# k2-fsa/Flow2GAN

Hardware: AMD Instinct MI355X
Metric: audio-seconds/sec (train step, G+D fwd/bwd) mel_24k_base (higher is better)
Workload: dtype f32 (fp32-class products on the bf16 matrix pipe for the long reductions and the direct MRD convs: every fp32 operand as three bf16 pieces = 24 significand bits, the six v_mfma_f32_32x32x16_bf16 products with i + j <= 2 per fp32 product, fp32 accumulate, error <= 2^-23 per product; short reductions ; 1 GPU; mel_24k_base GAN stage-2 train step: D-step + G-step, each on its own batch (MPD+MRD+FM+multi-scale mel), fwd+bwd+grad all-reduce, no optimizer (metric is fwd/bwd); per_gpu_batch=64, gan=gan_multi_scale_mel_recon, parallelism=dp1, optimizer=none

## Files before the change

flow2gan_amd/csrc/conv32x6.hip:

```cpp
#include <stdlib.h>

#include "conv32_common.h"

namespace {

typedef unsigned int u32x4 __attribute__((ext_vector_type(4)));

constexpr int NTAP = KH * KW;
constexpr int PB = 208;

__device__ __forceinline__ void split3(const f32x4 v, u32x2& p0, u32x2& p1, u32x2& p2) {
  unsigned a0, a1, a2, b0, b1, b2;
  f2g_split3_pair(v.x, v.y, a0, a1, a2);
  f2g_split3_pair(v.z, v.w, b0, b1, b2);
  p0 = u32x2{a0, b0};
  p1 = u32x2{a1, b1};
  p2 = u32x2{a2, b2};
}

__device__ __forceinline__ void store_px3(unsigned char* p, const f32x4 v) {
  u32x2 p0, p1, p2;
  split3(v, p0, p1, p2);
  *reinterpret_cast<u32x2*>(p) = p0;
  *reinterpret_cast<u32x2*>(p + 64) = p1;
// ... 502 lines not shown
      }
      if (row < XCH) split3(px_[row < XCH ? row : 0], kx[row < XCH ? row : 0][0], kx[row < XCH ? row : 0][1], kx[row < XCH ? row : 0][2]);
      if (row >= NK - GCH)
        split3(pg_[row >= NK - GCH ? row - (NK - GCH) : 0], kg[row >= NK - GCH ? row - (NK - GCH) : 0][0],
               kg[row >= NK - GCH ? row - (NK - GCH) : 0][1], kg[row >= NK - GCH ? row - (NK - GCH) : 0][2]);
    }
    {
      const int row = wave;
      bf16x8 a[3];
#pragma unroll
      for (int q = 0; q < 3; ++q) a[q] = tr_pix8(Gp + q * GPL + go + row * 16 * 64);
#pragma unroll
      for (int t = 0; t < 3; ++t) {
        bf16x8 b[3];
#pragma unroll
        for (int q = 0; q < 3; ++q) b[q] = tr_pix8(Xp + q * XPL + xs[t] + row * KR * IW * 64);
        mfma6(a, b, acc[3 + t]);
      }
    }
    __syncthreads();
    if (more) {
#pragma unroll
      for (int q = 0; q < XCH; ++q)
        if (xoff(q) >= 0) put3(Xp, XPL, xoff(q), kx[q]);
#pragma unroll
      for (int q = 0; q < GCH; ++q) put3(Gp, GPL, ((tid >> 3) + 64 * q) * 64 + c4 * 8, kg[q]);
    }
    __syncthreads();
  }
  static_assert(wgrad6_smem<TH, TW>() >= (size_t)8 * 16 * 64 * 4, "the flush reuses the planes as its reduction buffer");
  c32_wgrad_flush<NTAP, 3>(gw, reinterpret_cast<float*>(smb), acc, wave, lane, li, hh);
}

__global__ __launch_bounds__(512, 1) void conv33_x6_kernel(const f2g_conv32_desc d, int R, int tiles_h, int ntiles) {
  extern __shared__ __attribute__((aligned(16))) unsigned char smb[];
  unsigned char* At = smb;
  unsigned char* Bt = smb + P33 * PB;
  const int tid = threadIdx.x, lane = tid & 63, wave = tid >> 6;
  const int li = lane & 31, hh = lane >> 5;
  const int W = d.Win, PW = W + 2, npx = (R + 2) * PW, tpx = R * W;
  const unsigned mgW = magic_of(W), mgPW = magic_of(PW);
  {
    const unsigned char* wimg = reinterpret_cast<const unsigned char*>(d.w);
    for (int c = tid; c < T33 * C * 12; c += 512) {
      const int row = c / 12, part = c - row * 12;
      const int co = row / T33, tap = row - co * T33;
      *reinterpret_cast<u32x4*>(Bt + (tap * C + co) * PB + part * 16) =
          *reinterpret_cast<const u32x4*>(wimg + row * 192 + part * 16);
    }
  }
  constexpr int NQ = (P33 * 8 + 511) / 512;
  int prow[NQ], poff[NQ], pdst[NQ];
#pragma unroll
  for (int q = 0; q < NQ; ++q) {
    const int id = tid + 512 * q, px = id >> 3, c4 = id & 7;
    const int pr = fast_div(px, PW, mgPW), pc = px - pr * PW;
    const bool ok = px < npx && pc >= 1 && pc <= W;
    prow[q] = ok ? pr : -(1 << 20);
    poff[q] = (pr - 1) * (int)d.x_line + (pc - 1) * C + c4 * 4;
    pdst[q] = px < npx ? px * PB + c4 * 8 : -1;
  }
  auto load_patch = [&](int tile, f32x4 (&pf)[NQ]) {
    const int sq = tile / tiles_h, h0 = (tile - sq * tiles_h) * R;
    const float* org = d.x + (long long)sq * d.x_seq + (long long)h0 * d.x_line;
#pragma unroll
    for (int q = 0; q < NQ; ++q) {
      const int h = h0 - 1 + prow[q];
      pf[q] = *reinterpret_cast<const f32x4*>((h >= 0 && h < d.H) ? org + poff[q] : c32_zero);
    }
  };
  auto store_patch = [&](const f32x4 (&pf)[NQ]) {
#pragma unroll
    for (int q = 0; q < NQ; ++q)
      if (pdst[q] >= 0) store_px3(At + pdst[q], pf[q]);
  };
  const int mypx = wave * 32 + li;
  const int myr = fast_div(mypx, W, mgW), myc = mypx - myr * W;
  const unsigned char* Ap = At + (mypx < tpx ? ((myr + 1) * PW + myc + 1) * PB : (PW + 1) * PB) + hh * 16;
  const unsigned char* Bp = Bt + li * PB + hh * 16;
  const float bias = d.bias ? d.bias[li] : 0.f;
  float cs = 0.f;
  int tile = blockIdx.x;
  if (tile >= ntiles) return;
  {
    f32x4 pf[NQ];
    load_patch(tile, pf);
    store_patch(pf);
  }
  __syncthreads();
  for (; tile < ntiles; tile += gridDim.x) {
    const int nxt = tile + gridDim.x;
    const bool more = nxt < ntiles;
    f32x4 pf[NQ];
    load_patch(more ? nxt : tile, pf);
    const int sq = tile / tiles_h, h0 = (tile - sq * tiles_h) * R;
    const long long ybase = (long long)sq * d.y_seq + (long long)h0 * d.y_line;
    float my[16];
    if (d.mask_src) {
#pragma unroll
      for (int e = 0; e < 16; ++e) {
        const int p = wave * 32 + acc_row(e) + 4 * hh;
        const int r = fast_div(p, W, mgW), c = p - r * W;
        my[e] = (p < tpx && h0 + r < d.H) ? d.mask_src[ybase + (long long)r * d.y_line + c * C + li] : 1.f;
      }
    }
    f32x16 acc0, acc1;
#pragma unroll
    for (int e = 0; e < 16; ++e) { acc0[e] = 0.f; acc1[e] = 0.f; }
#pragma unroll
    for (int t = 0; t < T33; ++t)
      tap6(Ap + ((t / 3 - 1) * PW + (t % 3 - 1)) * PB, Bp + t * (C * PB), acc0, acc1);
    {
      float* ys = d.y + ybase;
#pragma unroll
      for (int e = 0; e < 16; ++e) {
        const int p = wave * 32 + acc_row(e) + 4 * hh;
        const int r = fast_div(p, W, mgW), c = p - r * W;
        if (p < tpx && h0 + r < d.H) {
          float v = acc0[e] + acc1[e] + bias;
          if (d.lrelu_slope != 0.f) v = v > 0.f ? v : d.lrelu_slope * v;
          if (d.mask_src) v *= my[e] > 0.f ? 1.f : d.mask_slope;
          cs += v;
          ys[(long long)r * d.y_line + c * C + li] = v;
        }
      }
    }
    __syncthreads();
    if (more) store_patch(pf);
    __syncthreads();
  }
  if (d.colsum) {
    cs += __shfl_xor(cs, 32);
    if (hh == 0) atomicAdd(d.colsum + li, cs);
  }
}


__global__ __launch_bounds__(512, 1) void conv33_wgrad6_kernel(const f2g_conv32_desc d, float* gw, int R,
                                                               int tiles_h, int ntiles) {
  extern __shared__ __attribute__((aligned(16))) unsigned char smb[];
  unsigned char* Xp = smb;
  unsigned char* Gp = smb + 3 * W33_XPL;
  const int tid = threadIdx.x, lane = tid & 63, wave = tid >> 6;
  const int li = lane & 31, hh = lane >> 5;
  const int W = d.Win, PW = W + 2, npx = (R + 2) * PW, ngp = R * PW, nks = (ngp + 15) >> 4;
  const unsigned mgPW = magic_of(PW);
  for (int o = tid * 16; o < 3 * (W33_XPL + W33_GPL); o += 512 * 16) *reinterpret_cast<u32x4*>(smb + o) = u32x4{0u, 0u, 0u, 0u};
  constexpr int NQ = (W33_GP * 8 + 511) / 512;
// ... 87 lines not shown
  const c32_tiling t = c32_pick_tiles(d->H, d->Wout);
  const long long nt = (long long)t.tiles_h * t.tiles_w * d->S;
  if (nt >= (1ll << 30) || d->x_line >= (1ll << 24)) return F2G_EINVAL;
  const int grid = (int)(nt < 256 ? nt : 256);
  return c32_launch_shape<conv32_s2_fwd6_kernel<8, 16>, conv32_s2_fwd6_kernel<16, 8>>(
      t.tall, fwd6_smem<8, 16>(), fwd6_smem<16, 8>(), dim3(grid), dim3(512), st, *d, t.tiles_w, t.tiles_h, (int)nt);
}

int f2g_conv32_dgrad6_launch(const f2g_conv32_desc* d, hipStream_t st) {
  const c32_tiling t = c32_pick_tiles(d->H, (d->Win + 1) / 2);
  const long long nt = (long long)t.tiles_h * t.tiles_w * d->S;
  if (nt >= (1ll << 30) || d->x_line >= (1ll << 24) || d->y_line >= (1ll << 24)) return F2G_EINVAL;
  const int grid = (int)(nt < 256 ? nt : 256);
  return c32_launch_shape<conv32_s2_dgrad6_kernel<8, 16>, conv32_s2_dgrad6_kernel<16, 8>>(
      t.tall, dgrad6_smem<8, 16>(), dgrad6_smem<16, 8>(), dim3(grid), dim3(512), st, *d, t.tiles_w, t.tiles_h,
      (int)nt);
}

int f2g_conv32_wgrad6_launch(const f2g_conv32_desc* d, float* gw, hipStream_t st) {
  const c32_tiling t = c32_pick_tiles(d->H, d->Wout);
  const long long nt = (long long)d->S * t.tiles_h * t.tiles_w;
  if (nt >= (1ll << 30) || d->x_line >= (1ll << 24)) return F2G_EINVAL;
  int per = (int)((nt + 255) / 256);
  if (per < 1) per = 1;
  const unsigned grid = (unsigned)((nt + per - 1) / per);
  return c32_launch_shape<conv32_s2_wgrad6_kernel<8, 16>, conv32_s2_wgrad6_kernel<16, 8>>(
      t.tall, wgrad6_smem<8, 16>(), wgrad6_smem<16, 8>(), dim3(grid), dim3(512), st, *d, gw, t.tiles_h, t.tiles_w,
      per);
}

int f2g_conv33_h3_launch(const f2g_conv32_desc* d, int R, int tiles_h, int ntiles, hipStream_t st);

extern "C" int f2g_conv33_fwd(const f2g_conv32_desc* d, f2g_stream_t stream) {
  if (!d || !d->x || !d->w || !d->y || (d->precision != 3 && d->precision != 4) || d->Win != d->Wout || d->fm_ref)
    return F2G_EINVAL;
  if ((((uintptr_t)d->x) & 15) || (((uintptr_t)d->w) & 15) || (d->x_line & 3) || (d->x_seq & 3)) return F2G_EINVAL;
  if (d->S <= 0 || d->H <= 0 || d->Win <= 0) return F2G_OK;
  const int W = d->Win;
  if (W > 112 || d->x_line >= (1ll << 24)) return F2G_EINVAL;
  if (d->y_line < (long long)W * C || (d->y != d->x && d->y_seq < (long long)d->H * d->y_line)) return F2G_EINVAL;
  if ((d->y_line & 3) || (d->y_seq & 3) || (((uintptr_t)d->y) & 15)) return F2G_EINVAL;
  if (d->mask_src && (d->lrelu_slope != 0.f || d->bias || (((uintptr_t)d->mask_src) & 15))) {
    f2g_set_error("f2g_conv33_fwd: mask_src (data-gradient role) excludes bias / lrelu_slope (forward role)");
    return F2G_EINVAL;
  }
  const int R = c33_pick_rows(d->H, W);
  if (R < 1) return F2G_EINVAL;
  const int tiles_h = (d->H + R - 1) / R;
  const long long nt = (long long)tiles_h * d->S;
  if (nt >= (1ll << 30)) return F2G_EINVAL;
  if (d->precision == 4) return f2g_conv33_h3_launch(d, R, tiles_h, (int)nt, (hipStream_t)stream);
  constexpr size_t smem = (size_t)P33 * PB + (size_t)T33 * C * PB;
  c32_lds_once<conv33_x6_kernel>(smem);
  const int grid = (int)(nt < 256 ? nt : 256);
  hipLaunchKernelGGL(conv33_x6_kernel, dim3(grid), dim3(512), smem, (hipStream_t)stream, *d, R, tiles_h, (int)nt);
  return f2g_check_launch();
}

extern "C" int f2g_conv33_wgrad(const f2g_conv32_desc* d, float* gw, f2g_stream_t stream) {
  if (!d || !d->x || !d->y || !gw || d->precision != 3 || d->Win != d->Wout) return F2G_EINVAL;
  if ((((uintptr_t)d->x) & 15) || (((uintptr_t)d->y) & 15) || (d->x_line & 3) || (d->x_seq & 3) || (d->y_line & 3) ||
      (d->y_seq & 3))
    return F2G_EINVAL;
  if (d->S <= 0 || d->H <= 0 || d->Win <= 0) return F2G_OK;
  const int W = d->Win;
  if (W > 112 || d->x_line >= (1ll << 24) || d->y_line >= (1ll << 24) || d->x_line < (long long)W * C ||
      d->y_line < (long long)W * C)
    return F2G_EINVAL;
  const int R = c33_pick_rows(d->H, W);
  if (R < 1) return F2G_EINVAL;
  const int tiles_h = (d->H + R - 1) / R;
  const long long nt = (long long)tiles_h * d->S;
  if (nt >= (1ll << 30)) return F2G_EINVAL;
  constexpr size_t smem = (size_t)3 * (W33_XPL + W33_GPL);
  static_assert(smem >= (size_t)8 * 16 * 64 * 4, "the flush reuses the planes as its reduction buffer");
  c32_lds_once<conv33_wgrad6_kernel>(smem);
  const int grid = (int)(nt < 256 ? nt : 256);
  hipLaunchKernelGGL(conv33_wgrad6_kernel, dim3(grid), dim3(512), smem, (hipStream_t)stream, *d, gw, R, tiles_h,
                     (int)nt);
  return f2g_check_launch();
}
```

flow2gan_amd/csrc/gemm_x6.hip:

```cpp
#include <stddef.h>
#include <stdint.h>

#include "gemm_common.h"
#include "x6_epilogue.h"

#define X6_MFMA_PRIO 1

#if F2G_X6LAB & 256
__device__ unsigned long long g_x6prof[8];
extern "C" int f2g_lab_x6prof(unsigned long long* out8) {
  unsigned long long z[8] = {0, 0, 0, 0, 0, 0, 0, 0};
  if (hipMemcpyFromSymbol(out8, HIP_SYMBOL(g_x6prof), sizeof(z)) != hipSuccess) return 1;
  return hipMemcpyToSymbol(HIP_SYMBOL(g_x6prof), z, sizeof(z)) != hipSuccess;
}
#endif

__global__ __launch_bounds__(256) void split3_img_kernel(__bf16* __restrict__ dst, const float* __restrict__ src,
                                                         long long ld, long long rows, int K) {
  const long long total = rows * (K / 4);
  for (long long i = (long long)blockIdx.x * blockDim.x + threadIdx.x; i < total;
       i += (long long)gridDim.x * blockDim.x) {
    const long long r = i / (K / 4);
    const int k4 = (int)(i - r * (K / 4)) * 4;
    const float4 v = *reinterpret_cast<const float4*>(src + r * ld + k4);
    const float x[4] = {v.x, v.y, v.z, v.w};
    unsigned short p[3][4];
#pragma unroll
    for (int e = 0; e < 4; ++e) {
      const __bf16 a = (__bf16)x[e];
      const float r1 = x[e] - (float)a;
      const __bf16 b = (__bf16)r1;
      const __bf16 c = (__bf16)(r1 - (float)b);
      p[0][e] = __builtin_bit_cast(unsigned short, a);
      p[1][e] = __builtin_bit_cast(unsigned short, b);
      p[2][e] = __builtin_bit_cast(unsigned short, c);
    }
// ... 518 lines not shown
#pragma unroll
    for (int ks = 0; ks < 2; ++ks)
#pragma unroll
      for (int sdeg = 2; sdeg >= 0; --sdeg)
#pragma unroll
        for (int i = 0; i < 3; ++i) {
          const int j = sdeg - i;
          if (j < 0 || j > 2) continue;
          acc[0][0] = __builtin_amdgcn_mfma_f32_32x32x16_bf16(fa[ks][i], fb[ks][j], acc[0][0], 0, 0, 0);
        }
  }
  const f2g_epilogue& E = d.E;
  if (E.aux || E.res || E.prelu_slope || E.atomic || E.accumulate || E.scale != 0.f) {
    gemm_epilogue<1, 1>(E, acc, M, N, m0, n0, wave, 0, li, h, true);
    return;
  }
  __syncthreads();
  long long* rowoff = reinterpret_cast<long long*>(smem6);
  if (tid < 128) {
    const int row = m0 + tid;
    long long off = -1;
    if (row < M) {
      if (E.P0o > 0) {
        const int sq = row / E.P0o;
        off = (long long)sq * E.seq_stride_o + (long long)(row - sq * E.P0o) * E.row_stride_o + E.off_o;
      } else {
        off = (long long)row * E.ldc;
      }
    }
    rowoff[tid] = off;
  }
  __syncthreads();
  const int col = li;
  if (col >= N) return;
  const float bias = E.bias ? E.bias[col] : 0.f;
  const float fmw = E.fm_ref ? E.fm_w * (E.fm_wdev ? E.fm_wdev[0] : 1.f) : 0.f;
  float cs = 0.f;
#pragma unroll
  for (int e = 0; e < 16; ++e) {
    const long long ro = rowoff[wave * 32 + (e & 3) + 8 * (e >> 2) + 4 * h];
    if (ro < 0) continue;
    const long long off = ro + col;
    float v = acc[0][0][e] + bias;
    if (E.lrelu_slope != 0.f) v = v > 0.f ? v : E.lrelu_slope * v;
    if (E.mask_src) {
      const float y = E.mask_src[off];
      if (E.fm_ref) {
        const float dl = y - E.fm_ref[off];
        v += fmw * (dl > 0.f ? 1.f : (dl < 0.f ? -1.f : 0.f));
      }
      v *= y > 0.f ? 1.f : E.mask_slope;
    }
    cs += v;
    E.C[off] = v;
  }
  if (E.colsum) {
    cs += __shfl_xor(cs, 32);
    if (h == 0) atomicAdd(E.colsum + col, cs);
  }
}


static bool x6_shape_ok(const f2g_gemm_desc& d) {
  if (d.form != 0 || !host_plain(d.B) || d.A.cols != d.B.cols) return false;
  const long long M = d.A.rows, N = d.B.rows, K = d.A.cols, ext = x6_a_extent(d.A);
  if (K < 32 || (K % 32) || M < 1 || N < 1 || ext <= 0) return false;
  if (ext * 6 >= 0xe0000000ll || N * K * 6 >= 0xe0000000ll) return false;
  if (d.A.alpha || d.A.lrelu_src || d.B.alpha || d.B.lrelu_src) return false;
  if (d.E.c_bf16 || d.E.atomic || d.split_k > 1) return false;
  if (d.E.x3_out) {
    const f2g_epilogue& E = d.E;
    if (E.prelu_out || (((uintptr_t)E.x3_out) & 15) || (((uintptr_t)E.C) & 15) || (N % 8)) return false;
    if (E.P0o > 0 ? ((E.seq_stride_o | E.row_stride_o | E.off_o) & 7) != 0 : (E.ldc & 7) != 0) return false;
  }
  return true;
}

static int x6_wide(const f2g_gemm_desc& d) {
  return x6e::wide_ok(d.E, d.B.rows) ? 1 : 0;
}

static bool x6f_ok(const f2g_gemm_desc& d) {
  if (d.A.split || (d.B.split != 0 && d.B.split != 3 && d.B.split != 4) || !x6_shape_ok(d)) return false;
  if (d.B.split == 4 && ((d.B.rows & 31) || d.B.rows <= 32 || d.B.P0 != 1 || d.B.P1 != 1)) return false;
  if (!al16(d.A.base) || !al16(d.B.base) || (d.A.seq_stride & 3) || (d.B.split == 0 && (d.B.seq_stride & 3))) return false;
  const long long ext = host_plain(d.A) ? (long long)d.A.rows * d.A.seq_stride : x6_a_extent(d.A);
  return ext * 4 < 0xe0000000ll && (long long)d.B.rows * (d.B.split ? d.B.cols * 6ll : d.B.seq_stride * 4) < 0xe0000000ll;
}

// ... 57 lines not shown
      f2g_note_kernel("x6n", 1, 5);
      hipLaunchKernelGGL(gemm_x6n_kernel, dim3((M + 127) / 128), dim3(256), smem_n, st, d, M, N, K, x6_rows_of(d.A, 4));
      break;
    }
    case X6_G: {
      constexpr size_t smem_g = 4 * x6e::ESZ > 128 * 208 ? 4 * x6e::ESZ : 128 * 208;
      f2g_note_kernel("x6g", 1, 4);
      hipLaunchKernelGGL(gemm_x6g_kernel, grid, dim3(256), smem_g, st, d, M, N, K, x6_rows_of(d.A, 4), x6_wide(d));
      break;
    }
    case X6_F:
      dyn_lds_once<gemm_x6f_kernel<false>, gemm_x6f_kernel<true>>((int)smem);
      f2g_note_kernel(pick.arg ? "x6f<wimg=1>" : "x6f<wimg=0>", 1, 4);
      hipLaunchKernelGGL(pick.arg ? gemm_x6f_kernel<true> : gemm_x6f_kernel<false>, grid, dim3(256), smem, st, d, M, N,
                         K, x6_rows_of(d.A, 4), x6_wide(d));
      break;
  }
  return f2g_check_launch();
}

extern "C" int f2g_gemm_x6_ok(const f2g_gemm_desc* d) {
  if (!d || !x6_shape_ok(*d)) return 0;
  return 1 | ((x6_tap_ok(*d, 5) || x6_tap_ok(*d, 2)) ? 2 : 0) | (x6f_ok(*d) ? 4 : 0);
}

extern "C" int32_t f2g_gemm_colsum_part_rows(const f2g_gemm_desc* dp) {
  if (!dp || (dp->precision != 3 && dp->precision != 4) || dp->form != 0) return 0;
  f2g_gemm_desc d = *dp;
  if (d.E.colsum_part_ld <= 0) d.E.colsum_part_ld = 4;
  if (d.precision == 4) {
    const int tile = f2g_gemm_h3_part_tile(d);
    return tile ? tile / 64 * ((d.A.rows + tile - 1) / tile) : 0;
  }
  if (!x6_wide(d)) return 0;
  const int M = d.A.rows;
  switch (x6_choose(d).kind) {
    case X6_NONE:
    case X6_N:
      return 0;
    case X6_P:
      return 4 * ((M + 255) / 256);
    default:
      return 2 * ((M + 127) / 128);
  }
}

extern "C" int64_t f2g_split_bf16x3_bytes(int32_t rows, int32_t K) { return (int64_t)rows * K * 6; }

extern "C" int f2g_split_bf16x3(void* dst, const float* src, int64_t ld, int32_t rows, int32_t K,
                                f2g_stream_t stream) {
  if (!dst || !src || rows < 0 || K < 32 || (K % 32) || ld < K || (ld & 3) || (((uintptr_t)src) & 15) ||
      (((uintptr_t)dst) & 15))
    return F2G_EINVAL;
  if (rows == 0) return F2G_OK;
  const long long total = (long long)rows * (K / 4);
  hipLaunchKernelGGL(split3_img_kernel, dim3(f2g_grid_for(total, 256)), dim3(256), 0, (hipStream_t)stream,
                     reinterpret_cast<__bf16*>(dst), src, (long long)ld, (long long)rows, K);
  return f2g_check_launch();
}
```

flow2gan_amd/csrc/thin_epilogue.h:

```cpp
#pragma once
#include "common.h"

namespace thin {

typedef float f32x16 __attribute__((ext_vector_type(16)));

__device__ __forceinline__ void row_offsets(const f2g_epilogue& E, int M, int m0, int tid, long long* rowoff) {
  if (tid >= 128) return;
  const int row = m0 + tid;
  long long off = -1;
  if (row < M) {
    if (E.P0o > 0) {
      const int sq = row / E.P0o;
      off = (long long)sq * E.seq_stride_o + (long long)(row - sq * E.P0o) * E.row_stride_o + E.off_o;
    } else {
      off = (long long)row * E.ldc;
    }
  }
  rowoff[tid] = off;
}

__device__ __forceinline__ float row_values(const f2g_epilogue& E, const f32x16& acc, int N, int wave, int li, int h,
                                            const long long* rowoff) {
  const int col = li;
// ... 24 lines not shown

__device__ __forceinline__ float row_values_cut(const f2g_epilogue& E, const f32x16& acc, int rg, int col0, int li,
                                                int h, const long long* rowoff, const int* rowlive) {
  const int col = col0 + li;
  float cs = 0.f;
  const float fmw = E.fm_ref ? E.fm_w * (E.fm_wdev ? E.fm_wdev[0] : 1.f) : 0.f;
#pragma unroll
  for (int e = 0; e < 16; ++e) {
    const int tr = rg * 32 + (e & 3) + 8 * (e >> 2) + 4 * h;
    const long long ro = rowoff[tr];
    if (ro < 0 || col >= rowlive[tr]) continue;
    const long long off = ro + col;
    float v = acc[e];
    if (E.mask_src) {
      const float y = E.mask_src[off];
      if (E.fm_ref) {
        const float dl = y - E.fm_ref[off];
        v += fmw * (dl > 0.f ? 1.f : (dl < 0.f ? -1.f : 0.f));
      }
      v *= y > 0.f ? 1.f : E.mask_slope;
    }
    cs += v;
    E.C[off] = v;
  }
  return cs;
}

__device__ __forceinline__ void column_sums(const f2g_epilogue& E, int N, int li, int h, float cs) {
  if (!E.colsum) return;
  cs += __shfl_xor(cs, 32);
  if (h == 0 && li < N) atomicAdd(E.colsum + li, cs);
}

}
```

flow2gan_amd/fused_disc.py:

```python
from __future__ import annotations

from typing import List

import torch

from . import ops
from .fused import deliver_grads, filterbank_spec, filterbank_spec_bwd, sink_register
from .models.modules import dft_matrices
from .ops import gemm, mat, win1d, win2d

SLOPE = 0.1


def stack_pair(real, fake):
    B, T = real.shape
    x2 = ops.empty(2 * B, T, device=real.device)
    ops.copy3(x2, 0, T, real.contiguous(), 0, T, 1, B, T)
    ops.copy3(x2, 0, T, fake.contiguous(), 0, T, 1, B, T, out_offset=B * T)
    return x2


def pack_conv_weight(w):
    Cout, Cin, kh, kw = w.shape
    out = ops.empty(Cout, kh * kw * Cin, device=w.device)
# ... 22 lines not shown
MPD_CH = (1, 32, 128, 512, 1024, 1024)
MPD_STRIDE = (3, 3, 3, 3, 1)


def mpd_params(mpd) -> list:
    p = []
    for d in mpd.discriminators:
        for c in d.convs:
            p += [c.weight, c.bias]
        p += [d.conv_post.weight, d.conv_post.bias]
    return p


HALO = 2


def _halo_rows(S: int, H: int, Cc: int, dev, x3: bool = False):
    buf = ops.empty(S * (H + 2 * HALO), Cc, device=dev)
    if Cc % 4 == 0:
        ops.zero_halo(buf, S, H + 2 * HALO, Cc, HALO, HALO)
    else:
        ops.fill_(buf, 0.0)
    if x3:
        ops.x3_reserve(buf, (S, H + 2 * HALO, Cc, HALO, HALO))
    return buf


def _halo_map(H: int, Cc: int):
    return (H, (H + 2 * HALO) * Cc, Cc, HALO * Cc)


def unhalo(y, S: int, H: int):
    return y.view(S, H + 2 * HALO, y.shape[1])[:, HALO:HALO + H]


def _mpd_forward_one(x2, p: int, prm: list, keep_images: bool = False):
    dev = x2.device
    S2, T = x2.shape
    H = (T + p - 1) // p
    S = S2 * p
    img = ops.empty(S * H, 1, device=dev)
    ops.period_fold(img, x2, S2, T, p, H)
    acts, hs = [img], [H]
    shares = [None] * 6
    x = img
    for l in range(5):
        w, b = prm[2 * l], prm[2 * l + 1]
        Cin, Cout, st = MPD_CH[l], MPD_CH[l + 1], MPD_STRIDE[l]
        Hout = (H + 4 - 5) // st + 1
        wp = ops.derived(w, "pack", pack_conv_weight)
        y = _halo_rows(S, Hout, Cout, dev, x3=(0 < l < 4))
        if l == 0:
            ops.mpd0_fwd(x, S, H, Hout, HALO, w.reshape(Cout, 5), b, SLOPE, y)
        else:
            A = win1d(x, S, H + 2 * HALO, Cin, Hout, st, 0, 5)
            if keep_images:
                shares[l] = ops.split_sharing(x)
                with shares[l]:
                    gemm(A, mat(wp), y, bias=b, lrelu=SLOPE, rowmap=_halo_map(Hout, Cout), x3_out=(l < 4))
            else:
                gemm(A, mat(wp), y, bias=b, lrelu=SLOPE, rowmap=_halo_map(Hout, Cout), x3_out=(l < 4))
        acts.append(y)
        hs.append(Hout)
        x, H = y, Hout
    wpost, bpost = prm[10], prm[11]
    wpp = ops.derived(wpost, "pack", pack_conv_weight)
    scores = ops.empty(S * H, 1, device=dev)
    ops.mpdpost_fwd(x, S, H, HALO, wpp, bpost, scores)
    return dict(acts=acts, hs=hs, scores=scores, S=S, p=p, shares=shares)


def _dgrad_weight(w, stride: int, j0: int, nt: int):
    def build(t):
        Cout, Cin, K = t.shape[0], t.shape[1], t.shape[2] * t.shape[3]
        out = ops.empty(Cin, nt * Cout, device=t.device)
        ops.permute4(out, t, (Cin, nt, Cout, 1), (K, -stride, Cin * K, 0),
                     in_offset=j0 + stride * (nt - 1))
        return out
    return ops.derived(w, ("dgradT", stride, j0, nt), build)


def _dgrad_weight3(w):
    def build(t):
        Cout, Cin, K = t.shape[0], t.shape[1], t.shape[2] * t.shape[3]
        out = ops.empty(3 * Cin, 2 * Cout, device=t.device)
        ops.fill_(out[:Cin], 0.0)
        one = ops.empty(Cin, Cout, device=t.device)
        ops.permute4(one, t, (Cin, 1, Cout, 1), (K, -3, Cin * K, 0), in_offset=2)
        ops.copy3(out, 2 * Cout, 0, one, Cout, 0, Cin, 1, Cout)
        for rho in (1, 2):
            ops.permute4(out[rho * Cin:(rho + 1) * Cin], t, (Cin, 2, Cout, 1), (K, -3, Cin * K, 0), in_offset=rho + 2)
        return out
    return ops.derived(w, ("dgradT3", 3), build)

# ... 9 lines not shown


def _conv1d_dgrad(g_pre, S, Hout, Cout, w, stride, pad, Hin, mask=None, fm=None, colsum=None):
    Cin, K = w.shape[1], w.shape[2] * w.shape[3]
    dev = g_pre.device
    want_img = 2 * Cin >= ops.X6_MIN_K
    gx = _halo_rows(S, Hin, Cin, dev, x3=want_img)
    if (K, stride, pad, Cin, Cout) == (5, 3, 2, 32, 128) and not want_img \
            and _conv1d_dgrad3(g_pre, S, Hout, Cout, w, Hin, gx, mask, fm, colsum):
        return gx
    for rho, j0, nt, e0, Lq in _residues(K, stride, pad, Hin):
        if Lq == 0:
            continue
        wq = _dgrad_weight(w, stride, j0, nt)
        wpad = (nt - 1) - e0
        A = win1d(g_pre, S, Hout + 2 * HALO, Cout, Lq, 1, wpad - HALO, nt)
        rm = (Lq, (Hin + 2 * HALO) * Cin, stride * Cin, (HALO + rho) * Cin)
        gemm(A, mat(wq), gx, rowmap=rm, mask=mask, fm=fm, colsum=colsum, x3_out=want_img)
    return gx


class MPDFusedLanding:

    def __init__(self, st, Sx: int, roff: int, g1, train_disc: bool):
        self.acts, self.hs, self.Sx, self.roff, self.g1, self.train_disc = st["acts"], st["hs"], Sx, roff, g1, train_disc

    def __call__(self, l_out, producer, cs):
        y, Sx, g1 = self.acts[l_out], self.Sx, self.g1
        Hp_, C_ = self.hs[l_out] + 2 * HALO, y.shape[1]
        mk = (y, self.roff * Hp_ * C_, SLOPE)
        fk = None
        if (not self.train_disc) and l_out >= 2:
            fk = (y, 0, 1.0 / (Sx * self.hs[l_out] * C_), g1)
        if l_out == 5 or (ops.GEMM_PRECISION == 3 and l_out in (3, 4)):
            return producer(mk, fk, cs)
        gm = producer(None, None, None)
        gm._f2g_x3_bad = True
        n_ = Sx * Hp_ * C_
        if self.train_disc:
            ops.lrelu_bwd_colsum(gm, y, None, 0.0, SLOPE, Sx * Hp_, C_, C_, cs, y_off=mk[1])
        elif fk is not None:
            ops.lrelu_bwd(gm, y, y, fk[2], SLOPE, 1, n_, n_, wdev=g1, y_off=mk[1], r_off=0)
        else:
            ops.lrelu_bwd(gm, y, None, 0.0, SLOPE, 1, n_, n_, y_off=mk[1])
        return gm


class MPDUpstreamLanding:

    def __init__(self, st, B: int, ups: dict):
        self.acts, self.hs, self.S, self.p, self.B, self.ups = st["acts"], st["hs"], st["S"], st["p"], B, ups

    def __call__(self, l_out, producer, cs):
        gm = producer(None, None, None)
        gm._f2g_x3_bad = True
        y, Hl, p = self.acts[l_out], self.hs[l_out], self.p
        Hp_, C_ = Hl + 2 * HALO, y.shape[1]
        u = self.ups.get(l_out)
        if u is not None:
            ub, uc, uh, uw = u.stride()
            ops.lrelu_bwd_add(gm, y, (self.B, p, Hl), (p * Hp_ * C_, Hp_ * C_, C_), C_, u, (ub, uw, uh, uc),
                              SLOPE, colsum=cs, g_off=HALO * C_)
        elif cs is not None:
            ops.lrelu_bwd_colsum(gm, y, None, 0.0, SLOPE, self.S * Hp_, C_, C_, cs)
        else:
            n_ = self.S * Hp_ * C_
            ops.lrelu_bwd(gm, y, None, 0.0, SLOPE, 1, n_, n_)
        return gm


# ... 233 lines not shown
                y = None
                gemm(A, mat(wp), cat, bias=b, lrelu=SLOPE,
                     rowmap=(Wout, Wcat * MRD_CH, MRD_CH, foff * MRD_CH))
            layer_out.append(y)
            x, x_is_spec = y, False
        acts.append(layer_out)
    wpost, bpost = prm[50], prm[51]
    scores = ops.empty(S * Ft * Wcat, 1, device=dev)
    w9 = ops.derived(wpost, "pack", pack_conv_weight)
    if ops.GEMM_PRECISION in (0, 1, 3):
        ops.convpost_fwd(cat, S, Ft, Wcat, w9, bpost, scores)
    else:
        gemm(win2d(cat, S, Ft, Wcat, MRD_CH, Wcat, 3, 3, 1, 1, 1), mat(w9), scores, bias=bpost)
    return dict(xn=xn, stats=stats, packed=packed, ldp=ldp, Ft=Ft, nb=nb, hop=hop, bands=bands,
                widths=widths, Wcat=Wcat, cat=cat, acts=acts, scores=scores)


def _conv2d_dgrad(g_pre, S, H, Wout, Cout, w, sw, Win, gx, *, g_line=None, g_seq=None, g_off=0,
                  x_line=None, x_off=0, mask=None, fm=None, colsum=None):
    Cin, kh, kw = w.shape[1], w.shape[2], w.shape[3]
    dev = g_pre.device
    pw = kw // 2
    if (ops.GEMM_PRECISION in (0, 1, 3) and Cin == MRD_CH and Cout == MRD_CH and kw == 9
            and sw == 2 and x_line is None and x_off == 0):
        def build_t(t):
            out = ops.empty(kh * kw, Cin, Cout, device=t.device)
            ops.permute4(out, t, (kh * kw, Cin, Cout, 1), (1, kh * kw, Cin * kh * kw, 0))
            return out
        wT = ops.derived(w, "dgrad_taps", build_t)
        ops.conv32_s2_dgrad(g_pre, S, H, Win, Wout, wT, gx, g_seq=g_seq, g_line=g_line, g_off=g_off,
                            mask=mask, fm=fm, colsum=colsum)
        return gx
    if (ops.GEMM_PRECISION == 3 and Cin == MRD_CH and Cout == MRD_CH
            and kh == 3 and kw == 3 and sw == 1 and x_line is None and x_off == 0 and fm is None
            and Win <= ops.CONV33_MAX_W):
        def build_f(t):
            out = ops.empty(Cin, kh * kw * Cout, device=t.device)
            ops.permute4(out, t, (Cin, kh * kw, Cout, 1), (kh * kw, -1, Cin * kh * kw, 0), in_offset=kh * kw - 1)
            return out
        wf = ops.derived(w, "dgrad33", build_f)
        ops.conv33(g_pre, S, H, Win, wf, None, 0.0, gx, x_off=g_off, x_line=g_line, x_seq=g_seq, form=1,
                   mask=mask, colsum=colsum)
        return gx
    if x_line is None:
        x_line = Win * Cin
    for rho, j0, ntw, e0, Lq in _residues(kw, sw, pw, Win):
        if Lq == 0:
            continue
        def build(t, j0=j0, ntw=ntw):
            out = ops.empty(kh * ntw * Cout, Cin, device=t.device)
            ops.permute4(out, t, (kh, ntw, Cout, Cin), (-kw, -sw, Cin * kh * kw, kh * kw),
                         in_offset=(kh - 1) * kw + j0 + sw * (ntw - 1))
            return out
        wq = ops.derived(w, ("dgrad2d", sw, j0, ntw), build)
        A = win2d(g_pre, S, H, Wout, Cout, Lq, kh, ntw, 1, 1, (ntw - 1) - e0, line_stride=g_line,
                  seq_stride=g_seq, offset=g_off)
        gemm(A, mat(wq), gx, form=1, rowmap=(Lq, x_line, sw * Cin, x_off + rho * Cin), mask=mask,
             fm=fm, colsum=colsum)
    return gx


def _mrd_foffs(st) -> list:
    foffs, foff = [], 0
    for ws in st["widths"]:
        foffs.append(foff)
        foff += ws[5]
    return foffs


class MRDFusedLanding:
    fused = True

    def __init__(self, st, Sx: int, soff: int, g1, train_disc: bool):
        self.st, self.Sx, self.soff, self.g1, self.train_disc = st, Sx, soff, g1, train_disc
        self.foffs = _mrd_foffs(st)

    def __call__(self, bi, l_out, producer, cs):
        st, Sx, soff, g1, train_disc = self.st, self.Sx, self.soff, self.g1, self.train_disc
        Ft, C = st["Ft"], MRD_CH
        Wl = st["widths"][bi][l_out + 1]
        if l_out == 4:
            gcat, cat, ldc, foff = producer(None, None, None), st["cat"], st["Wcat"] * C, self.foffs[bi]
            y_off = soff * Ft * ldc + foff * C
            if train_disc:
                ops.lrelu_bwd(gcat, cat, None, 0.0, SLOPE, Sx * Ft, Wl * C, ldc, g_off=foff * C, y_off=y_off)
            else:
                ops.lrelu_bwd(gcat, cat, cat, 1.0 / (Sx * Ft * Wl * C), SLOPE, Sx * Ft, Wl * C, ldc,
                              wdev=g1, g_off=foff * C, y_off=y_off, r_off=foff * C)
            return gcat
        yb = st["acts"][bi][l_out]
        nb_ = Sx * Ft * Wl * C
        mk = (yb, soff * Ft * Wl * C, SLOPE)
        fmk = (yb, 0, 1.0 / nb_, g1) if ((not train_disc) and l_out >= 1) else None
        if (train_disc and ops.GEMM_PRECISION == 3 and ops.CONV32_X6
                and (l_out < 3 or Wl <= ops.CONV33_MAX_W)):
            return producer(mk, fmk, cs)
        gx = producer(None, None, None)
        if train_disc:
            ops.lrelu_bwd_colsum(gx, yb, None, 0.0, SLOPE, Sx * Ft * Wl, C, C, cs, y_off=mk[1])
        elif fmk is not None:
            ops.lrelu_bwd(gx, yb, yb, fmk[2], SLOPE, 1, nb_, nb_, wdev=g1, y_off=mk[1], r_off=0)
        else:
            ops.lrelu_bwd(gx, yb, None, 0.0, SLOPE, 1, nb_, nb_, y_off=mk[1])
        return gx


class MRDUpstreamLanding:
    fused = False

    def __init__(self, st, S: int, g_maps):
        self.st, self.S, self.g_maps = st, S, g_maps
        self.foffs = _mrd_foffs(st)

    def __call__(self, bi, l_out, producer, cs):
        st, S = self.st, self.S
        Ft, C = st["Ft"], MRD_CH
        Wl = st["widths"][bi][l_out + 1]
        gm = producer(None, None, None)
        u = self.g_maps[4 * bi + l_out - 1] if l_out >= 1 else None
        if l_out == 4:
            y, line, off = st["cat"], st["Wcat"] * C, self.foffs[bi] * C
        else:
            y, line, off = st["acts"][bi][l_out], Wl * C, 0
        if u is not None:
            ub, uc, uf, uw = u.stride()
            ops.lrelu_bwd_add(gm, y, (S, Ft, Wl), (Ft * line, line, C), C, u, (ub, uf, uw, uc), SLOPE,
                              colsum=cs, g_off=off)
        elif l_out == 4:
            ops.lrelu_bwd(gm, y, None, 0.0, SLOPE, S * Ft, Wl * C, line, g_off=off, y_off=off)
            if cs is not None:
# ... 272 lines not shown
```

flow2gan_amd/ops.py:

```python
from __future__ import annotations

import ctypes as C
from typing import Callable, NamedTuple, Optional

import torch

from . import _lib as L
from ._opts import opt
from ._lib import DwconvBwd, DwnormBwd, DwnormFwd, Epilogue, GemmDesc, Operand, call, ptr


def empty(*shape, device, dtype=torch.float32):
    return torch.empty(*shape, device=device, dtype=dtype)


def zeros(*shape, device):
    t = torch.empty(*shape, device=device, dtype=torch.float32)
    fill_(t, 0.0)
    return t


def fill_(t, v: float):
    if BATCH is not None and t.numel() > 0:
        import struct
# ... 910 lines not shown
            continue
        d.precision = 4
        if mark_a:
            d.A.split = mark_a
        if mark_b:
            d.B.split = mark_b
        ask = lambda: L.lib.f2g_gemm_f16_ok(C.byref(d)) == needs
        if _ask_with_x3_out(d, out, out_offset, x3_out, prelu_out, ask) if wide else ask():
            return r
        if mark_a or mark_b:
            d.A.split = d.B.split = 0
    return None


def _fp16x3_gemm(d, A, Bm, out, form: int, atomic: bool, split_k: int, out_offset: int, x3_out: bool,
                 prelu_out) -> bool:
    r = _fp16x3_route(d, A, Bm, out, form, atomic, split_k, out_offset, x3_out, prelu_out)
    if r is None:
        return False
    image_a, image_b = r.images
    new_a = image_a(A) if image_a is not None else None
    new_b = image_b(Bm) if image_b is not None else None
    if new_a is not None:
        d.A = new_a
    if new_b is not None:
        d.B = new_b
    globals()[r.counter] += 1
    if x3_out and r.x3_out and d.E.x3_out:
        out._f2g_x3 = out._f2g_x3_buf
    return True


CONV32_X6 = opt("conv32_x6", True)


def x3_image(t2d):
    def build(t):
        rows, K = t.shape
        img = torch.empty(rows * K * 3, device=t.device, dtype=torch.bfloat16)
        split3(img, t, 0, K, rows, K)
        return img
    return derived(t2d, "x3img", build) if _is_const(t2d) else build(t2d)


def _timed_conv(name, flops, shape, *args):
    if GEMM_TIMER is not None:
        GEMM_TIMER.time(lambda: call(name, *args), flops, shape)
    else:
        call(name, *args)


FP16X3_CONV32_FWD = opt("fp16x3_conv32_fwd", False)
FP16X3_CONV32_DGRAD = opt("fp16x3_conv32_dgrad", False)
FP16X3_CONV32_WGRAD = opt("fp16x3_conv32_wgrad", False)
FP16X3_CONV33_FWD = opt("fp16x3_conv33_fwd", False)
FP16X3_CONV33_DGRAD = opt("fp16x3_conv33_dgrad", False)
FP16X3_CONV33_WGRAD = opt("fp16x3_conv33_wgrad", False)
FP16X3_CONV32_FWD_LAUNCHES = 0
FP16X3_CONV32_DGRAD_LAUNCHES = 0
FP16X3_CONV32_WGRAD_LAUNCHES = 0
FP16X3_CONV33_FWD_LAUNCHES = 0
FP16X3_CONV33_DGRAD_LAUNCHES = 0
FP16X3_CONV33_WGRAD_LAUNCHES = 0


def conv32_f16_image(w):
# ... 4 lines not shown

def _conv32_operand(d, w, rows_k=None, h3: bool = False):
    img = w
    if GEMM_PRECISION == 1:
        d.precision = 1
        img = derived(w, "split", split_bf16) if w is not None else None
    elif GEMM_PRECISION == 3 and CONV32_X6:
        if h3 and FP16X3 and w is not None:
            d.precision = 4
            img = conv32_f16_image(w)
        else:
            d.precision = 3
            img = x3_image(w.view(rows_k) if rows_k else w) if w is not None else None
    if img is not w:
        d._keep = img
    return img


def conv32_s2_fwd(x, S: int, H: int, Win: int, Wout: int, w_packed, bias, slope: float, y):
    global FP16X3_CONV32_FWD_LAUNCHES
    d = L.Conv32Desc()
    d.x, d.x_seq, d.x_line = ptr(x), H * Win * 32, Win * 32
    d.S, d.H, d.Win, d.Wout = S, H, Win, Wout
    d.w, d.bias, d.lrelu_slope = ptr(_conv32_operand(d, w_packed, h3=FP16X3_CONV32_FWD)), ptr(bias), slope
    FP16X3_CONV32_FWD_LAUNCHES += d.precision == 4
    d.y, d.y_seq, d.y_line = ptr(y), H * Wout * 32, Wout * 32
    _timed_conv("f2g_conv32_s2_fwd", 2.0 * S * H * Wout * 32 * 27 * 32, (0, S * H * Wout, 32, 27 * 32), C.byref(d))
    return y


CONV33_MAX_W = 112


def conv33(x, S: int, H: int, W: int, w_packed, bias, slope: float, y, x_off: int = 0, x_line=None, x_seq=None,
           y_off: int = 0, y_line=None, y_seq=None, form: int = 0, mask=None, colsum=None):
    global FP16X3_CONV33_FWD_LAUNCHES, FP16X3_CONV33_DGRAD_LAUNCHES
    d = L.Conv32Desc()
    d.x = ptr(x) + 4 * x_off
    d.x_line = x_line if x_line is not None else W * 32
    d.x_seq = x_seq if x_seq is not None else H * d.x_line
    d.S, d.H, d.Win, d.Wout = S, H, W, W
    if FP16X3 and GEMM_PRECISION == 3 and CONV32_X6 and (FP16X3_CONV33_DGRAD if form == 1 else FP16X3_CONV33_FWD):
        img = conv32_f16_image(w_packed)
        d.precision = 4
        if form == 1:
            FP16X3_CONV33_DGRAD_LAUNCHES += 1
        else:
            FP16X3_CONV33_FWD_LAUNCHES += 1
    else:
        img = x3_image(w_packed)
        d.precision = 3
    d._keep = img
    d.w, d.bias, d.lrelu_slope = ptr(img), ptr(bias), slope
    d.y = ptr(y) + 4 * y_off
    d.y_line = y_line if y_line is not None else W * 32
    d.y_seq = y_seq if y_seq is not None else H * d.y_line
    if mask is not None:
        d.mask_src = ptr(mask[0]) + 4 * mask[1]
        d.mask_slope = float(mask[2])
    d.colsum = ptr(colsum)
    _timed_conv("f2g_conv33_fwd", 2.0 * S * H * W * 32 * 9 * 32, (form, S * H * W, 32, 9 * 32), C.byref(d))
    return y


def conv33_wgrad(x, g, S: int, H: int, W: int, gw, g_off: int = 0, g_line=None, g_seq=None):
    global FP16X3_CONV33_WGRAD_LAUNCHES
    d = L.Conv32Desc()
    d.x, d.x_line, d.x_seq = ptr(x), W * 32, H * W * 32
    d.S, d.H, d.Win, d.Wout = S, H, W, W
    d.precision = 3
    d.y = ptr(g) + 4 * g_off
    d.y_line = g_line if g_line is not None else W * 32
    d.y_seq = g_seq if g_seq is not None else H * d.y_line
    name = "f2g_conv33_wgrad"
    if FP16X3 and GEMM_PRECISION == 3 and CONV32_X6 and FP16X3_CONV33_WGRAD:
        d.precision = 4
        name = "f2g_conv33_wgrad_h3"
        FP16X3_CONV33_WGRAD_LAUNCHES += 1
    _timed_conv(name, 2.0 * S * H * W * 32 * 9 * 32, (2, 32, 9 * 32, S * H * W), C.byref(d), ptr(gw))
    return gw


def conv32_s2_dgrad(g, S: int, H: int, Win: int, Wout: int, wT, gx, g_seq=None, g_line=None,
                    g_off: int = 0, mask=None, fm=None, colsum=None):
    global FP16X3_CONV32_DGRAD_LAUNCHES
    d = L.Conv32Desc()
    d.x = ptr(g) + 4 * g_off
    d.x_line = g_line if g_line is not None else Wout * 32
    d.x_seq = g_seq if g_seq is not None else H * d.x_line
    d.S, d.H, d.Win, d.Wout = S, H, Win, Wout
    wT = _conv32_operand(d, wT, (27 * 32, 32), h3=FP16X3_CONV32_DGRAD)
    FP16X3_CONV32_DGRAD_LAUNCHES += d.precision == 4
# ... 889 lines not shown
```

Measured before the change: 809.4 audio-s/s.

## Fuse feature-matching and LReLU-mask landing into MRD/MPD backward conv epilogues

Measured after the change: 817.0 audio-s/s (median of 6 runs). About the same (+0.9%).

```diff
diff --git a/flow2gan_amd/csrc/conv32x6.hip b/flow2gan_amd/csrc/conv32x6.hip
--- a/flow2gan_amd/csrc/conv32x6.hip
+++ b/flow2gan_amd/csrc/conv32x6.hip
@@ -558,6 +558,7 @@
   c32_wgrad_flush<NTAP, 3>(gw, reinterpret_cast<float*>(smb), acc, wave, lane, li, hh);
 }
 
+template <bool FM>
 __global__ __launch_bounds__(512, 1) void conv33_x6_kernel(const f2g_conv32_desc d, int R, int tiles_h, int ntiles) {
   extern __shared__ __attribute__((aligned(16))) unsigned char smb[];
   unsigned char* At = smb;
@@ -606,6 +607,16 @@
   const unsigned char* Bp = Bt + li * PB + hh * 16;
   const float bias = d.bias ? d.bias[li] : 0.f;
   float cs = 0.f;
+  const float fmw = FM ? d.fm_w * (d.fm_wdev ? d.fm_wdev[0] : 1.f) : 0.f;
+  int eo[FM ? 16 : 1];
+  if constexpr (FM) {
+#pragma unroll
+    for (int e = 0; e < 16; ++e) {
+      const int p = wave * 32 + acc_row(e) + 4 * hh;
+      const int r = fast_div(p, W, mgW), c = p - r * W;
+      eo[e] = r * (int)d.y_line + c * C + li;
+    }
+  }
   int tile = blockIdx.x;
   if (tile >= ntiles) return;
   {
@@ -621,8 +632,16 @@
     load_patch(more ? nxt : tile, pf);
     const int sq = tile / tiles_h, h0 = (tile - sq * tiles_h) * R;
     const long long ybase = (long long)sq * d.y_seq + (long long)h0 * d.y_line;
-    float my[16];
-    if (d.mask_src) {
+    float my[16], fr[FM ? 16 : 1];
+    const int np = (d.H - h0 < R ? d.H - h0 : R) * W;
+    if constexpr (FM) {
+#pragma unroll
+      for (int e = 0; e < 16; ++e) {
+        const bool in = wave * 32 + acc_row(e) + 4 * hh < np;
+        my[e] = in ? d.mask_src[ybase + eo[e]] : 1.f;
+        fr[e] = in ? d.fm_ref[ybase + eo[e]] : 0.f;
+      }
+    } else if (d.mask_src) {
 #pragma unroll
       for (int e = 0; e < 16; ++e) {
         const int p = wave * 32 + acc_row(e) + 4 * hh;
@@ -640,6 +659,14 @@
       float* ys = d.y + ybase;
 #pragma unroll
       for (int e = 0; e < 16; ++e) {
+        if constexpr (FM) {
+          if (wave * 32 + acc_row(e) + 4 * hh < np) {
+            const float v = c32_mask_fm(acc0[e] + acc1[e], my[e], true, [&] { return fr[e]; }, fmw, d.mask_slope);
+            cs += v;
+            ys[eo[e]] = v;
+          }
+          continue;
+        }
         const int p = wave * 32 + acc_row(e) + 4 * hh;
         const int r = fast_div(p, W, mgW), c = p - r * W;
         if (p < tpx && h0 + r < d.H) {
@@ -793,8 +820,12 @@
 int f2g_conv33_h3_launch(const f2g_conv32_desc* d, int R, int tiles_h, int ntiles, hipStream_t st);
 
 extern "C" int f2g_conv33_fwd(const f2g_conv32_desc* d, f2g_stream_t stream) {
-  if (!d || !d->x || !d->w || !d->y || (d->precision != 3 && d->precision != 4) || d->Win != d->Wout || d->fm_ref)
+  if (!d || !d->x || !d->w || !d->y || (d->precision != 3 && d->precision != 4) || d->Win != d->Wout)
     return F2G_EINVAL;
+  if (d->fm_ref && (d->precision != 3 || !d->mask_src || (((uintptr_t)d->fm_ref) & 15) || d->y_line >= (1ll << 22))) {
+    f2g_set_error("f2g_conv33_fwd: fm_ref needs mask_src, precision 3 and y_line < 2^22");
+    return F2G_EINVAL;
+  }
   if ((((uintptr_t)d->x) & 15) || (((uintptr_t)d->w) & 15) || (d->x_line & 3) || (d->x_seq & 3)) return F2G_EINVAL;
   if (d->S <= 0 || d->H <= 0 || d->Win <= 0) return F2G_OK;
   const int W = d->Win;
@@ -812,9 +843,16 @@
   if (nt >= (1ll << 30)) return F2G_EINVAL;
   if (d->precision == 4) return f2g_conv33_h3_launch(d, R, tiles_h, (int)nt, (hipStream_t)stream);
   constexpr size_t smem = (size_t)P33 * PB + (size_t)T33 * C * PB;
-  c32_lds_once<conv33_x6_kernel>(smem);
   const int grid = (int)(nt < 256 ? nt : 256);
-  hipLaunchKernelGGL(conv33_x6_kernel, dim3(grid), dim3(512), smem, (hipStream_t)stream, *d, R, tiles_h, (int)nt);
+  if (d->fm_ref) {
+    c32_lds_once<conv33_x6_kernel<true>>(smem);
+    hipLaunchKernelGGL(conv33_x6_kernel<true>, dim3(grid), dim3(512), smem, (hipStream_t)stream, *d, R, tiles_h,
+                       (int)nt);
+  } else {
+    c32_lds_once<conv33_x6_kernel<false>>(smem);
+    hipLaunchKernelGGL(conv33_x6_kernel<false>, dim3(grid), dim3(512), smem, (hipStream_t)stream, *d, R, tiles_h,
+                       (int)nt);
+  }
   return f2g_check_launch();
 }
 
diff --git a/flow2gan_amd/csrc/gemm_x6.hip b/flow2gan_amd/csrc/gemm_x6.hip
--- a/flow2gan_amd/csrc/gemm_x6.hip
+++ b/flow2gan_amd/csrc/gemm_x6.hip
@@ -2,6 +2,7 @@
 #include <stdint.h>
 
 #include "gemm_common.h"
+#include "thin_epilogue.h"
 #include "x6_epilogue.h"
 
 #define X6_MFMA_PRIO 1
@@ -586,14 +587,15 @@
   }
   __syncthreads();
   const int col = li;
-  if (col >= N) return;
-  const float bias = E.bias ? E.bias[col] : 0.f;
+  const bool parts = E.colsum_part_ld > 0 && E.colsum;
+  if (col >= N && !parts) return;
+  const float bias = (E.bias && col < N) ? E.bias[col] : 0.f;
   const float fmw = E.fm_ref ? E.fm_w * (E.fm_wdev ? E.fm_wdev[0] : 1.f) : 0.f;
   float cs = 0.f;
 #pragma unroll
   for (int e = 0; e < 16; ++e) {
     const long long ro = rowoff[wave * 32 + (e & 3) + 8 * (e >> 2) + 4 * h];
-    if (ro < 0) continue;
+    if (ro < 0 || col >= N) continue;
     const long long off = ro + col;
     float v = acc[0][0][e] + bias;
     if (E.lrelu_slope != 0.f) v = v > 0.f ? v : E.lrelu_slope * v;
@@ -608,7 +610,9 @@
     cs += v;
     E.C[off] = v;
   }
-  if (E.colsum) {
+  if (parts) {
+    thin::column_sums_part(E, N, blockIdx.x, wave, li, h, cs, reinterpret_cast<float*>(smem6 + 128 * sizeof(long long)));
+  } else if (E.colsum) {
     cs += __shfl_xor(cs, 32);
     if (h == 0) atomicAdd(E.colsum + col, cs);
   }
@@ -732,9 +736,16 @@
     const int tile = f2g_gemm_h3_part_tile(d);
     return tile ? tile / 64 * ((d.A.rows + tile - 1) / tile) : 0;
   }
+  const int M = d.A.rows;
+  const x6_kind kind = x6_choose(d).kind;
+  if (kind == X6_N) {
+    const f2g_epilogue& E = d.E;
+    if (E.aux || E.res || E.prelu_slope || E.atomic || E.accumulate || E.scale != 0.f || E.colsum_alpha)
+      return 0;
+    return (M + 127) / 128;
+  }
   if (!x6_wide(d)) return 0;
-  const int M = d.A.rows;
-  switch (x6_choose(d).kind) {
+  switch (kind) {
     case X6_NONE:
     case X6_N:
       return 0;
diff --git a/flow2gan_amd/csrc/thin_epilogue.h b/flow2gan_amd/csrc/thin_epilogue.h
--- a/flow2gan_amd/csrc/thin_epilogue.h
+++ b/flow2gan_amd/csrc/thin_epilogue.h
@@ -80,4 +80,13 @@
   if (h == 0 && li < N) atomicAdd(E.colsum + li, cs);
 }
 
+__device__ __forceinline__ void column_sums_part(const f2g_epilogue& E, int N, int tile, int wave, int li, int h,
+                                                 float cs, float* part) {
+  cs += __shfl_xor(cs, 32);
+  if (h == 0) part[wave * 32 + li] = cs;
+  __syncthreads();
+  if (wave == 0 && h == 0 && li < N)
+    E.colsum[(long long)tile * E.colsum_part_ld + li] = (part[li] + part[32 + li]) + (part[64 + li] + part[96 + li]);
 }
+
+}
diff --git a/flow2gan_amd/fused_disc.py b/flow2gan_amd/fused_disc.py
--- a/flow2gan_amd/fused_disc.py
+++ b/flow2gan_amd/fused_disc.py
@@ -78,6 +78,12 @@
 
 def unhalo(y, S: int, H: int):
     return y.view(S, H + 2 * HALO, y.shape[1])[:, HALO:HALO + H]
+
+
+def mpd_wants_image(l: int, Cout: int) -> bool:
+    if not 0 < l < 4:
+        return False
+    return 5 * Cout >= ops.X6_MIN_K or not ops.MPD_LEAN_IMAGES
 
 
 def _mpd_forward_one(x2, p: int, prm: list, keep_images: bool = False):
@@ -95,7 +101,7 @@
         Cin, Cout, st = MPD_CH[l], MPD_CH[l + 1], MPD_STRIDE[l]
         Hout = (H + 4 - 5) // st + 1
         wp = ops.derived(w, "pack", pack_conv_weight)
-        y = _halo_rows(S, Hout, Cout, dev, x3=(0 < l < 4))
+        y = _halo_rows(S, Hout, Cout, dev, x3=mpd_wants_image(l, Cout))
         if l == 0:
             ops.mpd0_fwd(x, S, H, Hout, HALO, w.reshape(Cout, 5), b, SLOPE, y)
         else:
@@ -103,9 +109,11 @@
             if keep_images:
                 shares[l] = ops.split_sharing(x)
                 with shares[l]:
-                    gemm(A, mat(wp), y, bias=b, lrelu=SLOPE, rowmap=_halo_map(Hout, Cout), x3_out=(l < 4))
-            else:
-                gemm(A, mat(wp), y, bias=b, lrelu=SLOPE, rowmap=_halo_map(Hout, Cout), x3_out=(l < 4))
+                    gemm(A, mat(wp), y, bias=b, lrelu=SLOPE, rowmap=_halo_map(Hout, Cout),
+                         x3_out=mpd_wants_image(l, Cout))
+            else:
+                gemm(A, mat(wp), y, bias=b, lrelu=SLOPE, rowmap=_halo_map(Hout, Cout),
+                     x3_out=mpd_wants_image(l, Cout))
         acts.append(y)
         hs.append(Hout)
         x, H = y, Hout
@@ -181,10 +189,12 @@
         fk = None
         if (not self.train_disc) and l_out >= 2:
             fk = (y, 0, 1.0 / (Sx * self.hs[l_out] * C_), g1)
-        if l_out == 5 or (ops.GEMM_PRECISION == 3 and l_out in (3, 4)):
+        if l_out == 5 or (ops.GEMM_PRECISION == 3 and l_out in (3, 4)) \
+                or (ops.MPD_LAND_FUSED and ops.GEMM_PRECISION == 3 and not ops.FP16X3 and l_out in (1, 2)):
             return producer(mk, fk, cs)
         gm = producer(None, None, None)
         gm._f2g_x3_bad = True
+        ops.LANDING_PASSES += 1
         n_ = Sx * Hp_ * C_
         if self.train_disc:
             ops.lrelu_bwd_colsum(gm, y, None, 0.0, SLOPE, Sx * Hp_, C_, C_, cs, y_off=mk[1])
@@ -484,15 +494,15 @@
                             mask=mask, fm=fm, colsum=colsum)
         return gx
     if (ops.GEMM_PRECISION == 3 and Cin == MRD_CH and Cout == MRD_CH
-            and kh == 3 and kw == 3 and sw == 1 and x_line is None and x_off == 0 and fm is None
-            and Win <= ops.CONV33_MAX_W):
+            and kh == 3 and kw == 3 and sw == 1 and x_line is None and x_off == 0
+            and (fm is None or ops.conv33_fm_ok()) and Win <= ops.CONV33_MAX_W):
         def build_f(t):
             out = ops.empty(Cin, kh * kw * Cout, device=t.device)
             ops.permute4(out, t, (Cin, kh * kw, Cout, 1), (kh * kw, -1, Cin * kh * kw, 0), in_offset=kh * kw - 1)
             return out
         wf = ops.derived(w, "dgrad33", build_f)
         ops.conv33(g_pre, S, H, Win, wf, None, 0.0, gx, x_off=g_off, x_line=g_line, x_seq=g_seq, form=1,
-                   mask=mask, colsum=colsum)
+                   mask=mask, fm=fm, colsum=colsum)
         return gx
     if x_line is None:
         x_line = Win * Cin
@@ -534,6 +544,7 @@
         if l_out == 4:
             gcat, cat, ldc, foff = producer(None, None, None), st["cat"], st["Wcat"] * C, self.foffs[bi]
             y_off = soff * Ft * ldc + foff * C
+            ops.LANDING_PASSES += 1
             if train_disc:
                 ops.lrelu_bwd(gcat, cat, None, 0.0, SLOPE, Sx * Ft, Wl * C, ldc, g_off=foff * C, y_off=y_off)
             else:
@@ -544,10 +555,11 @@
         nb_ = Sx * Ft * Wl * C
         mk = (yb, soff * Ft * Wl * C, SLOPE)
         fmk = (yb, 0, 1.0 / nb_, g1) if ((not train_disc) and l_out >= 1) else None
-        if (train_disc and ops.GEMM_PRECISION == 3 and ops.CONV32_X6
-                and (l_out < 3 or Wl <= ops.CONV33_MAX_W)):
+        if (ops.GEMM_PRECISION == 3 and ops.CONV32_X6 and (l_out < 3 or Wl <= ops.CONV33_MAX_W)
+                and (train_disc or (ops.MRD_LAND_FUSED_G and (fmk is None or l_out < 3 or ops.conv33_fm_ok())))):
             return producer(mk, fmk, cs)
         gx = producer(None, None, None)
+        ops.LANDING_PASSES += 1
         if train_disc:
             ops.lrelu_bwd_colsum(gx, yb, None, 0.0, SLOPE, Sx * Ft * Wl, C, C, cs, y_off=mk[1])
         elif fmk is not None:
diff --git a/flow2gan_amd/ops.py b/flow2gan_amd/ops.py
--- a/flow2gan_amd/ops.py
+++ b/flow2gan_amd/ops.py
@@ -966,6 +966,10 @@
 
 
 CONV32_X6 = opt("conv32_x6", True)
+MRD_LAND_FUSED_G = opt("mrd_land_fused_g", True)
+MPD_LAND_FUSED = opt("mpd_land_fused", True)
+MPD_LEAN_IMAGES = opt("mpd_lean_images", True)
+LANDING_PASSES = 0
 
 
 def x3_image(t2d):
@@ -1036,15 +1040,24 @@
 CONV33_MAX_W = 112
 
 
+def _conv33_h3(form: int) -> bool:
+    return bool(FP16X3 and GEMM_PRECISION == 3 and CONV32_X6
+                and (FP16X3_CONV33_DGRAD if form == 1 else FP16X3_CONV33_FWD))
+
+
+def conv33_fm_ok() -> bool:
+    return not _conv33_h3(1)
+
+
 def conv33(x, S: int, H: int, W: int, w_packed, bias, slope: float, y, x_off: int = 0, x_line=None, x_seq=None,
-           y_off: int = 0, y_line=None, y_seq=None, form: int = 0, mask=None, colsum=None):
+           y_off: int = 0, y_line=None, y_seq=None, form: int = 0, mask=None, fm=None, colsum=None):
     global FP16X3_CONV33_FWD_LAUNCHES, FP16X3_CONV33_DGRAD_LAUNCHES
     d = L.Conv32Desc()
     d.x = ptr(x) + 4 * x_off
     d.x_line = x_line if x_line is not None else W * 32
     d.x_seq = x_seq if x_seq is not None else H * d.x_line
     d.S, d.H, d.Win, d.Wout = S, H, W, W
-    if FP16X3 and GEMM_PRECISION == 3 and CONV32_X6 and (FP16X3_CONV33_DGRAD if form == 1 else FP16X3_CONV33_FWD):
+    if _conv33_h3(form):
         img = conv32_f16_image(w_packed)
         d.precision = 4
         if form == 1:
@@ -1062,6 +1075,8 @@
     if mask is not None:
         d.mask_src = ptr(mask[0]) + 4 * mask[1]
         d.mask_slope = float(mask[2])
+        if fm is not None:
+            d.fm_ref, d.fm_w, d.fm_wdev = ptr(fm[0]) + 4 * fm[1], float(fm[2]), ptr(fm[3])
     d.colsum = ptr(colsum)
     _timed_conv("f2g_conv33_fwd", 2.0 * S * H * W * 32 * 9 * 32, (form, S * H * W, 32, 9 * 32), C.byref(d))
     return y
```
